# Yuval-H/iclr_17_compression

Hardware: AMD Instinct MI355X
Metric: Mpixels/s encode+decode at 1/2/4/8 GPU; bpp & PSNR parity on Kodak (higher is better)
Workload: dtype h3; 1 GPU; eval encode+decode (round quantiser + rate), 64 x 256x256x3 images per GPU, N=192; N=192, image=256x256x3, batch_per_gpu=64, global_batch=64, quant=round, parallelism=dp1 (images sharded by rank, no data-path collective), launch=eager (kernel by kernel)

## Files before the change

iclr_17_compression_amd/csrc/engine_h3.hip:

```cpp
#include <stdio.h>
#include <stdlib.h>
#include <string.h>

#include <atomic>
#include <type_traits>

#include "common.h"
#include "k5_common.h"

namespace iclr17 {
namespace h3k {
using namespace bfm;

__device__ __attribute__((aligned(16))) unsigned g_zero16h[4] = {0u, 0u, 0u, 0u};
__device__ __forceinline__ const void* zero16(int) { return g_zero16h; }

__device__ __forceinline__ void sink4(void* lds_sink) {
  __builtin_amdgcn_global_load_lds((const __attribute__((address_space(1))) void*)g_zero16h,
                                   (__attribute__((address_space(3))) void*)lds_sink, 4, 0, 0);
}

__device__ __forceinline__ f16v mfma32h(const u4& a, const u4& b, const f16v& c) {
  return __builtin_amdgcn_mfma_f32_32x32x16_f16(__builtin_bit_cast(h8v, a),
                                                __builtin_bit_cast(h8v, b), c, 0, 0, 0);
}

enum HEpi : int { HE_GDN = 0, HE_IGDN = 1, HE_QUANT = 2 };

struct HArgs {
  const u16* in;
  const float* img;
  long in_plane;
  const u16* w;
  long w_plane;
  const float* wscale;
  const float* bias;
  const float* beta;
  const u16* gamma_h3;
  const float* gamma_scale;
  float* out;
  float* pre;
  u16* out_h3;
  long out_h3_plane;
  u16* out_x6;
  long out_x6_plane;
  int out_cm;
  int* range;
  int* wide;
  int qmode;
  const float* noise;
  const float* rate;
  const float* rtab;
  float* yhat;
  double* partial;
  int T;
  int B, Hin, Win, Hout, Wout;
  int gh, gw;
  int tiles_x, tiles_y;
};

constexpr int HM_CONV8 = 2;
constexpr int kConv8Steps = 13;

template <int TH>
struct PatchC8 {
  static constexpr int ROWS = 2 * TH + 3;
  static constexpr int ROWB = 640;
  static constexpr int BYTES = ROWS * ROWB;
  __host__ __device__ static constexpr int off(int pr, int pc) {
    return pr * ROWB + (pc & 1) * 320 + (pc >> 1) * 16;
  }
  __host__ __device__ static constexpr int tap8(int t) {
    return t < 25 ? off(t / 5, t % 5) : 0;
  }
};
constexpr int HM_CONV1 = 3;
constexpr int kConv1Steps = 16;
template <int TH>
struct PatchC1 {
  static constexpr int ROWS = 4 * TH + 5;
  static constexpr int ROWB = 160;
  static constexpr int BYTES = 3 * ROWS * ROWB;
  __host__ __device__ static constexpr int rowoff(int g) { return ((g / 9) * ROWS + g % 9) * ROWB; }
  __host__ __device__ static constexpr int gath(int q) {
    return q < 27 ? ((q / 9) * ROWS + q % 9) * ROWB + 16 : -1;
  }
};

template <int MODE, int TH>
struct HPatch {
  using type = Patch<MODE, TH>;
};
template <int TH>
struct HPatch<HM_CONV8, TH> {
  using type = PatchC8<TH>;
};
template <int TH>
struct HPatch<HM_CONV1, TH> {
  using type = PatchC1<TH>;
};

template <int MODE, int TH, int CO, int CI, bool INT_IN, int NS = 4>
struct HK {
  static constexpr int NW = TH / 2, NTHR = NW * 64;
  static constexpr int NT = CO / 32;
  static constexpr bool C1 = MODE == HM_CONV1;
  static constexpr int CCH = MODE == HM_CONV8 ? 8 : 16;
  static constexpr int NCH = C1 ? 1 : CI / CCH;
  using P = typename HPatch<MODE, TH>::type;
  static constexpr int PL = INT_IN ? 1 : 2;
  static constexpr int PB = PL * P::BYTES;
  static constexpr int NQI = C1 ? 0 : (PB + 1023) / 1024;
  static constexpr int PBUF = (PB + 1023) / 1024 * 1024;
  static constexpr int NPB = C1 ? 1 : 2;
  static constexpr int SB = 2 * 2 * CO * 16;
  static constexpr int NBI = SB / 1024;
  static constexpr int NST = NS;
  static constexpr int MAIN = NPB * PBUF + NST * SB + 1024;
  static constexpr int NTH = NT / 2;
  static constexpr int KB = CO / 16;
  static constexpr int GBL = 2 * NTH * KB;
  static constexpr int LDS0 = MAIN > GBL * 1024 ? MAIN : GBL * 1024;
  static constexpr int BBOFF = (LDS0 + 1023) / 1024 * 1024;
  static constexpr int LDS = BBOFF + 2048 + 256;
  static_assert(SB % 1024 == 0, "weight stage");
  static_assert(C1 || CI % CCH == 0, "tile shape");
  static_assert(LDS <= 160 * 1024, "LDS");
};

__device__ __forceinline__ long h3_out_off(const HArgs& a, int b, int oy, int ox, int CO, int ch) {
  const int cm = a.out_cm;
  if (cm == 0) return (((long)b * a.Hout + oy) * a.Wout + ox) * CO + ch;
  const int sh = __builtin_ctz(cm);
  return ((((long)b * (CO >> sh) + (ch >> sh)) * a.Hout + oy) * a.Wout + ox << sh) + (ch & (cm - 1));
}
__device__ __forceinline__ long h3_out_step32(const HArgs& a) {
  return a.out_cm == 0 ? 32L : 32L * a.Hout * a.Wout;
}

template <int TH, int CO, int COT>
__device__ __forceinline__ void quant_epilogue(const HArgs& a, f16v (&acc)[COT / 32],
                                               unsigned char* lds0, unsigned char* scratch, int b,
                                               int ty, int tx, int cg) {
  constexpr int NT = COT / 32, NW = TH / 2;
  const int etid = fresh_tid(), elane = etid & 63, er32 = elane & 31, eh = elane >> 5;
  const int ewave = __builtin_amdgcn_readfirstlane(etid >> 6);
  const int gy = ty * TH + 2 * ewave + (er32 >> 4), gx = tx * 16 + (er32 & 15);
  const bool inside = gy < a.gh && gx < a.gw;
  const long o = ((long)b * a.Hout + gy) * a.Wout + gx;
  const float dsc = a.wscale[1];
  const bool round = a.qmode == ICLR17_QUANT_ROUND;
  const bool table = a.rtab != nullptr && round;
  float* const lq = (float*)lds0 + etid * 32;
  float bits = 0.f;
  bool ovf = false, wid = false;
  const bool poison = a.range != nullptr && (*(const volatile int*)a.range & 1) != 0;
#pragma unroll
  for (int i = 0; i < NT; ++i) {
    const int c0 = cg * COT + 32 * i;
    float q[16], bv[16];
    bool slow = false;
#pragma unroll
    for (int r = 0; r < 16; ++r) {
      const int c = c0 + 8 * (r >> 2) + 4 * eh + (r & 3);
      const float y = poison ? __builtin_nanf("") : acc[i][r] * dsc;
      acc[i][r] = y;
      const float yh = round ? rintf(y)
                             : y + (inside ? a.noise[(((long)b * CO + c) * a.Hout + gy) * a.Wout + gx] : 0.f);
      q[r] = yh;
      bv[r] = table ? a.rtab[c * 65 + (int)fminf(fmaxf(yh, -32.f), 32.f) + 32] : 0.f;
      slow |= inside && !(table && fabsf(yh) <= 32.f);
    }
    if (slow) {
#pragma unroll
      for (int r = 0; r < 16; ++r) lq[r] = q[r];
#pragma unroll 1
      for (int r = 0; r < 16; ++r) {
        const float v = lq[r];
        if (!(table && fabsf(v) <= 32.f))
          lq[16 + r] = element_bits(v, a.rate, CO, c0 + 8 * (r >> 2) + 4 * eh + (r & 3));
      }
#pragma unroll
      for (int r = 0; r < 16; ++r)
        if (!(table && fabsf(q[r]) <= 32.f)) bv[r] = lq[16 + r];
    }
#pragma unroll
    for (int r = 0; r < 16; ++r) bits += inside ? bv[r] : 0.f;
    f4 yq[4];
#pragma unroll
    for (int m = 0; m < 4; ++m) {
      yq[m] = f4{q[4 * m], q[4 * m + 1], q[4 * m + 2], q[4 * m + 3]};
      if (inside) {
        *(f4*)(a.yhat + o * CO + c0 + 8 * m + 4 * eh) = yq[m];
        if (a.out)
          *(f4*)(a.out + o * CO + c0 + 8 * m + 4 * eh) =
              f4{acc[i][4 * m], acc[i][4 * m + 1], acc[i][4 * m + 2], acc[i][4 * m + 3]};
      }
    }
    if (a.out_h3) {
      uint2 hb[4], lb[4];
      bool ov = false, wd = false;
#pragma unroll
      for (int m = 0; m < 4; ++m) h3_split4(yq[m], hb[m], lb[m], ov, wd);
      ovf |= inside && ov;
      wid |= inside && wd;
      u4 sv[2][2];
#pragma unroll
      for (int pl = 0; pl < 2; ++pl)
#pragma unroll
        for (int k = 0; k < 2; ++k) {
          const uint2 A = pl ? lb[k] : hb[k], Bv = pl ? lb[k + 2] : hb[k + 2];
          const auto sx = __builtin_amdgcn_permlane32_swap(A.x, Bv.x, false, false);
          const auto sy = __builtin_amdgcn_permlane32_swap(A.y, Bv.y, false, false);
          sv[pl][k] = u4{sx[0], sy[0], sx[1], sy[1]};
        }
      if (inside) {
        const long s0 = h3_out_off(a, b, gy, gx, CO, c0 + 16 * eh);
        const long s1 = h3_out_off(a, b, gy, gx, CO, c0 + 16 * eh + 8);
        *(u4*)(a.out_h3 + s0) = sv[0][0];
        *(u4*)(a.out_h3 + s1) = sv[0][1];
        *(u4*)(a.out_h3 + a.out_h3_plane + s0) = sv[1][0];
        *(u4*)(a.out_h3 + a.out_h3_plane + s1) = sv[1][1];
      }
    }
  }
  if (ovf && a.range) atomicOr(a.range, 2);
  if (wid && a.wide) atomicOr(a.wide, 1);
  bits = wave_sum(poison ? __builtin_nanf("") : bits);
  float* sw = (float*)scratch;
  if (elane == 0) sw[ewave] = bits;
  __syncthreads();
  if (etid == 0) {
    double t = 0.0;
#pragma unroll
    for (int w = 0; w < NW; ++w) t += (double)sw[w];
    a.partial[(long)b * a.T + (ty * a.tiles_x + tx) * (CO / COT) + cg] = t;
  }
}

template <int MODE, int TH, int CO, int CI, int EPI, bool INT_IN, int PH, int COT = CO,
          bool SEP = false, int ICM = 0>
__device__ __forceinline__ void h3k_body(const HArgs& a, unsigned char* smem, int b, int ty, int tx,
                                         int cg, bool narrow) {
  static_assert(CO % COT == 0 && (COT == CO || EPI == HE_QUANT), "channel groups: conv3 only");
  constexpr int NSG = EPI == HE_QUANT ? 6 : 4;
  using KK = HK<MODE, TH, COT, CI, INT_IN, NSG>;
  using P = typename KK::P;
  constexpr bool CONV = MODE != BM_DECONV, C8 = MODE == HM_CONV8, C1 = MODE == HM_CONV1;
  using TP = Taps<CONV ? BM_CONV : BM_DECONV, PH>;
  constexpr int NT = KK::NT, NW = KK::NW, NCH = KK::NCH;
  constexpr int S = C1 ? kConv1Steps : C8 ? kConv8Steps : TP::T;
  constexpr int SB = KK::SB, NBI = KK::NBI, NST = KK::NST;
  const int tid = threadIdx.x, lane = tid & 63;
  const int wave = __builtin_amdgcn_readfirstlane(tid >> 6);
  const int r32 = lane & 31, h = lane >> 5;
  constexpr int F = NSG - 2 < S - 1 ? NSG - 2 : (S >= 3 ? 2 : 1), SI = S - F;
  static_assert(SI >= 1 && NST >= F + 2, "DMA schedule");
  constexpr int PS = (KK::NQI + SI - 1) / SI;
  constexpr int K = (NBI + PS + NW - 1) / NW;
  static_assert(F * K < 64, "vmcnt");
  constexpr int GS = NCH * S;
  unsigned char* const sP = smem;
  unsigned char* const sB = smem + KK::NPB * KK::PBUF;
  unsigned char* const sD = sB + NST * SB;
  float* const sbb = (float*)(smem + KK::BBOFF);
  const long img = (long)b * a.Hin * a.Win;
  const int iy0 = CONV ? 2 * ty * TH - 2 : ty * TH - 1;
  const int ix0 = CONV ? 2 * tx * 16 - 2 : tx * 16 - 1;
  static_assert(ICM == 0 || ICM == KK::CCH, "chunk-major input: one chunk per layout chunk");
  const long cstride = ICM ? (long)a.Hin * a.Win * ICM : KK::CCH;
  constexpr int PXS = ICM ? ICM : CI;
  const u16* __restrict__ inb = a.in + img * CI;
  auto piece_src = [&](int piece) -> long {
    const int byte = (piece * 64 + lane) * 16;
    const int pl = byte / P::BYTES, rem = byte - pl * P::BYTES;
    const int pr = rem / P::ROWB, r1 = rem - pr * P::ROWB;
    int pc, hh = 0;
    bool ok;
    if constexpr (C1) {
      pc = 0;
      ok = false;
    } else if constexpr (C8) {
      const int par = r1 / 320, slot = (r1 - par * 320) / 16;
      pc = 2 * slot + par;
      ok = slot < 18 && pc < 35;
    } else if constexpr (MODE == BM_CONV) {
      const int par = r1 / (2 * P::HALF), r2 = r1 - par * 2 * P::HALF;
      hh = r2 / P::HALF;
      pc = 2 * ((r2 - hh * P::HALF) / 16) + par;
      ok = pc < 35;
    } else {
      hh = r1 / P::HALF;
      pc = (r1 - hh * P::HALF) / 16;
      ok = true;
    }
    const int iy = iy0 + pr, ix = ix0 + pc;
    ok = ok && pl < KK::PL && (unsigned)iy < (unsigned)a.Hin && (unsigned)ix < (unsigned)a.Win;
    return ok ? pl * a.in_plane + (long)(iy * a.Win + ix) * PXS + 8 * hh : -1;
  };
  auto issue_piece = [&](int c1, int piece, bool valid) {
    if (!valid) {
      sink4(sD);
      return;
    }
    const long src = piece_src(piece);
    glds16(src >= 0 ? (const void*)(inb + src + c1 * cstride) : zero16(lane),
           sP + (c1 & 1) * KK::PBUF + piece * 1024);
  };
  constexpr long WSTEP = 2L * CO * 8;
  const u16* __restrict__ wph = a.w;
  if (MODE == BM_DECONV) {
    long off = 0;
#pragma unroll
    for (int p = 0; p < PH; ++p) {
      const int ny = (p >> 1) == 0 ? 3 : 2, nx = (p & 1) == 0 ? 3 : 2;
      off += (long)NCH * ny * nx * WSTEP;
    }
    wph += off;
  }
  int wsrc[K];
#pragma unroll
  for (int k = 0; k < K; ++k) {
    const int q = (k * NW + wave) * 64 + lane;
    const int pl = q / (2 * COT), u = q - pl * (2 * COT), hu = u / COT;
    wsrc[k] = (int)(pl * a.w_plane) + (hu * CO + cg * COT + (u - hu * COT)) * 8;
  }
  auto issue_w = [&](int k, int wg) {
    const int slot = k * NW + wave;
    if (wg >= GS) {
      sink4(sD);
      return;
    }
    glds16(wph + (long)wg * WSTEP + wsrc[k], sB + (wg % NST) * SB + slot * 1024);
  };

  const int prow = 2 * wave + (r32 >> 4), pcol = r32 & 15;
  const int tpix = prow * 16 + pcol;
  int pbase;
  if constexpr (C1) pbase = 4 * prow * P::ROWB + 8 * pcol;
  else if constexpr (C8) pbase = P::off(2 * prow, 2 * pcol);
  else pbase = (MODE == BM_CONV ? P::off(2 * prow, 2 * pcol) : P::off(prow, pcol)) + h * P::HALF;
  auto tap_of = [&](int s) -> int {
    if constexpr (C8) return h ? P::tap8(2 * s + 1) : P::tap8(2 * s);
    else if constexpr (C1) return 0;
    else return P::template tap_off<PH>(s);
  };
  const int abase = (h * COT + r32) * 16;
  constexpr int APL = 2 * COT * 16;

  f16v acc[NT], cacc[NT];
#pragma unroll
  for (int i = 0; i < NT; ++i)
#pragma unroll
    for (int j = 0; j < 16; ++j) acc[i][j] = 0.f;

  static_assert(CO <= 256, "bias / β stage");
  if (EPI != HE_QUANT && wave < 2) {
    const float* src = wave == 0 ? a.bias : a.beta;
    glds16(lane * 4 < CO ? (const void*)(src + lane * 4) : zero16(lane), sbb + wave * 256);
  }
  for (int piece = wave; piece < KK::NQI; piece += NW) issue_piece(0, piece, true);
#pragma unroll
  for (int f = 0; f < F; ++f)
#pragma unroll
    for (int k = 0; k < K; ++k)
      if (k * NW + wave < NBI) issue_w(k, f);
#pragma unroll
  for (int k = 0; k < K; ++k) {
    if (k * NW + wave < NBI) issue_w(k, F);
    else sink4(sD);
  }
#pragma unroll
  for (int f = 1; f < F; ++f)
#pragma unroll
    for (int k = 0; k < K; ++k) sink4(sD);
  if constexpr (C1) {
    constexpr int QR = 18, NU = 3 * P::ROWS * QR, IT = (NU + KK::NTHR - 1) / KK::NTHR;
    const int jy0 = 4 * TH * ty - 4, jx0 = 64 * tx - 4;
    const float* __restrict__ xb = a.img + (long)b * 3 * a.Hin * a.Win;
    f4 v[IT];
#pragma unroll
    for (int it = 0; it < IT; ++it) {
      const int u = tid + it * KK::NTHR;
      const int q = u % QR, cr = u / QR, c = cr / P::ROWS, r = cr - c * P::ROWS;
      const int iy = jy0 + r, ix = jx0 + 4 * q;
      const bool ok = u < NU && (unsigned)iy < (unsigned)a.Hin && (unsigned)ix < (unsigned)a.Win;
      v[it] = ok ? *(const f4*)(xb + ((long)c * a.Hin + iy) * a.Win + ix) : f4{0.f, 0.f, 0.f, 0.f};
    }
    bool povf = false;
#pragma unroll
    for (int it = 0; it < IT; ++it) {
      const int u = tid + it * KK::NTHR;
      if (u >= NU) break;
      const int q = u % QR, cr = u / QR;
      uint2 hb, lb;
      h3_split4(v[it], hb, lb, povf);
      *(uint2*)(sP + cr * P::ROWB + 8 * q) = hb;
      *(uint2*)(sP + P::BYTES + cr * P::ROWB + 8 * q) = lb;
    }
    if (povf && a.range) atomicOr(a.range, 1);
    __builtin_amdgcn_s_waitcnt(0xC07F);
  }

  typedef const __attribute__((address_space(3))) u4* lu4p;
  auto dma_k = [&](int k, int c, int s, int g) {
    const int slot = k * NW + wave;
    if ((k + 1) * NW <= NBI || slot < NBI) {
      issue_w(k, g + F + 1);
    } else if (s < SI) {
      const int piece = s * PS + slot - NBI;
      issue_piece(c + 1, piece, c + 1 < NCH && piece < KK::NQI);
    } else {
      sink4(sD);
    }
  };
  struct Frag {
    u4 bh, bl, wh[NT], wl[NT];
  };
  typedef unsigned u2e __attribute__((ext_vector_type(2)));
  typedef const __attribute__((address_space(3))) u2e* lu2p;
  typedef const __attribute__((address_space(3))) unsigned short* lu16p;
  auto conv1_b = [&](const unsigned char* pp, int s) -> u4 {
    u4 v = u4{0u, 0u, 0u, 0u};
    if constexpr (!C1) return v;
    else {
    const int g0 = 2 * s, g1 = 2 * s + 1;
    if (g0 < 27) {
      const int ro = h ? (g1 < 27 ? P::rowoff(g1) : P::rowoff(g0)) : P::rowoff(g0);
      const u2e x0 = *(lu2p)(pp + ro), x1 = *(lu2p)(pp + ro + 8);
      v = u4{x0.x, x0.y, x1.x, x1.y};
    }
    if (g1 >= 27) {
      unsigned e[8];
#pragma unroll
      for (int j = 0; j < 8; ++j) {
        const int oa = g0 >= 27 ? P::gath(8 * (g0 - 27) + j) : -1;
        const int ob = P::gath(8 * (g1 - 27) + j);
        const int o = h ? ob : oa;
        const unsigned x = *(lu16p)(pp + (o >= 0 ? o : 0));
        e[j] = o >= 0 ? x : 0u;
      }
      const u4 w = u4{e[0] | (e[1] << 16), e[2] | (e[3] << 16), e[4] | (e[5] << 16), e[6] | (e[7] << 16)};
      if (g0 >= 27) v = w;
      else if (h) v = w;
    }
    return v;
    }
  };
  auto read_frag = [&](Frag& f, const unsigned char* pb, int to, const unsigned char* wb, int s) {
    if constexpr (C1) {
      f.bh = conv1_b(sP + pbase, s);
      f.bl = conv1_b(sP + P::BYTES + pbase, s);
    } else {
      f.bh = *(lu4p)(pb + to);
      if constexpr (!INT_IN) f.bl = *(lu4p)(pb + P::BYTES + to);
      else f.bl = u4{0u, 0u, 0u, 0u};
    }
#pragma unroll
    for (int i = 0; i < NT; ++i) {
      f.wh[i] = *(lu4p)(wb + i * 512);
      f.wl[i] = *(lu4p)(wb + APL + i * 512);
    }
  };
  auto main_loop = [&](auto narrow_form) {
  constexpr bool NARROW = decltype(narrow_form)::value;
  Frag cur;
  int stage = 1;
  for (int c = 0; c < NCH; ++c) {
    if constexpr (SEP) {
#pragma unroll
      for (int i = 0; i < NT; ++i)
#pragma unroll
        for (int j = 0; j < 16; ++j) cacc[i][j] = 0.f;
    }
#pragma unroll
    for (int s = 0; s < S; ++s) {
      const int g = c * S + s;
      wait_vm_barrier<(F - 1) * K>();
      if (s == 0 && c == 0) read_frag(cur, sP + pbase, tap_of(0), sB + abase, 0);
      Frag nxt;
      read_frag(nxt, sP + ((s + 1 < S ? c : c + 1) & 1) * KK::PBUF + pbase,
                tap_of(s + 1 < S ? s + 1 : 0), sB + stage * SB + abase, s + 1 < S ? s + 1 : 0);
      stage = stage + 1 == NST ? 0 : stage + 1;
      u4 bh11 = cur.bh;
      if constexpr (NARROW) bh11 = h3_x2048(cur.bh);
#pragma unroll
      for (int i = 0; i < NT; ++i) {
        f16v t = SEP ? cacc[i] : acc[i];
        if constexpr (!INT_IN) t = mfma32h(cur.wh[i], cur.bl, t);
        t = mfma32h(cur.wl[i], cur.bh, t);
        if constexpr (NARROW) t = mfma32h(cur.wh[i], bh11, t);
        else t = mfma32h(h3_x2048(cur.wh[i]), cur.bh, t);
        if constexpr (SEP) cacc[i] = t;
        else acc[i] = t;
      }
#pragma unroll
      for (int k = 0; k < K; ++k) dma_k(k, c, s, g);
      cur = nxt;
    }
    if constexpr (SEP) {
#pragma unroll
      for (int i = 0; i < NT; ++i) acc[i] += cacc[i];
    }
  }
  };
  if (!C1 && __builtin_amdgcn_readfirstlane((int)narrow)) main_loop(std::true_type{});
  else main_loop(std::false_type{});
  vm_barrier();
  if constexpr (EPI == HE_QUANT) {
    using KF = HK<MODE, TH, COT, CI, false, NSG>;
    static_assert(TH / 2 * 64 * 128 <= KF::BBOFF, "the epilogue's lane rows fit the stages");
    quant_epilogue<TH, CO, COT>(a, acc, smem, smem + KF::BBOFF, b, ty, tx, cg);
    return;
  } else {

  const int etid = fresh_tid(), elane = etid & 63, er32 = elane & 31, eh = elane >> 5;
  const int ewave = __builtin_amdgcn_readfirstlane(etid >> 6);
  const int etpix = (2 * ewave + (er32 >> 4)) * 16 + (er32 & 15);
  const int gy = ty * TH + (etpix >> 4), gx = tx * 16 + (etpix & 15);
  const bool inside = gy < a.gh && gx < a.gw;
  const int oy = CONV ? gy : 2 * gy + (PH >> 1);
  const int ox = CONV ? gx : 2 * gx + (PH & 1);
  const long o = ((long)b * a.Hout + oy) * a.Wout + ox;
  const float dsc = a.wscale[1];
  const long hb0 = h3_out_off(a, b, oy, ox, CO, 16 * eh), hb1 = h3_out_off(a, b, oy, ox, CO, 16 * eh + 8);
  const long hstep = h3_out_step32(a);
#pragma unroll
  for (int i = 0; i < NT; ++i)
#pragma unroll
    for (int m = 0; m < 4; ++m) {
      const f4 bv = *(const f4*)(sbb + 32 * i + 8 * m + 4 * eh);
#pragma unroll
      for (int j = 0; j < 4; ++j) acc[i][4 * m + j] = acc[i][4 * m + j] * dsc + bv[j];
    }
  constexpr int NTH = KK::NTH, KB = KK::KB;
  static_assert(NT % 2 == 0, "GDN epilogue: pairs of 32-channel tiles");
  bool ovf = false, wid = false;
  float mx = 0.f;
#pragma unroll
  for (int i = 0; i < NT; ++i)
#pragma unroll
    for (int j = 0; j < 16; ++j) mx = fmaxf(mx, fabsf(acc[i][j]));
  mx = fmaxf(mx, __shfl_xor(mx, 32, 64));
  int ep = 0;
  {
    const float m2 = mx * mx;
    if (m2 > 0.f && m2 <= 3.40282347e38f) {
      int e;
      frexpf(m2, &e);
      ep = 14 - e < 100 ? 14 - e : 100;
    }
  }
  const float sp = ldexpf(1.0f, ep);
  const float nsc = ldexpf(a.gamma_scale[1] * kH3Sa, -ep);
  constexpr int KH = KB / 2, HBL = 2 * NTH * KH, GK = (HBL + NW - 1) / NW;
  static_assert(KB % 2 == 0 && 2 * HBL * 1024 <= KK::LDS0, "γ half-stages");
  auto stage_g = [&](int q) {
    const int hf = q >> 1, kh = q & 1;
#pragma unroll
    for (int k = 0; k < GK; ++k) {
      const int blk = k * NW + ewave;
      if (blk >= HBL) {
        sink4((unsigned char*)sbb + 2048);
        continue;
      }
      const int p = blk / (NTH * KH), rem = blk - p * NTH * KH;
      const int il = rem / KH, kb = kh * KH + rem - il * KH;
      glds16(a.gamma_h3 + (long)p * CO * CO + ((2 * kb + eh) * CO + 32 * (hf * NTH + il) + er32) * 8,
             smem + (q & 1) * HBL * 1024 + blk * 1024);
    }
  };
  stage_g(0);
  stage_g(1);
#pragma unroll
  for (int hf = 0; hf < 2; ++hf) {
#pragma unroll
    for (int i = 0; i < NT; ++i)
#pragma unroll
      for (int j = 0; j < 16; ++j) asm volatile("" : "+v"(acc[i][j]));
    f16v n[NTH];
#pragma unroll
    for (int il = 0; il < NTH; ++il)
#pragma unroll
      for (int j = 0; j < 16; ++j) n[il][j] = 0.f;
#pragma unroll
    for (int kh = 0; kh < 2; ++kh) {
      const int q = 2 * hf + kh;
      if (q == 0) {
        wait_vm_barrier<GK>();
      } else {
        vm_barrier();
        if (q + 1 < 4 && q >= 1) stage_g(q + 1);
      }
      const unsigned char* sg = smem + (q & 1) * HBL * 1024 + elane * 16;
#pragma unroll
      for (int kk = 0; kk < KH; ++kk) {
        const int kb = kh * KH + kk;
        const int i = kb >> 1, r0 = 8 * (kb & 1);
        unsigned hv[4], lv[4];
#pragma unroll
        for (int qq = 0; qq < 4; ++qq) {
          typedef float f2 __attribute__((ext_vector_type(2)));
          const f2 v = f2{acc[i][r0 + 2 * qq] * acc[i][r0 + 2 * qq], acc[i][r0 + 2 * qq + 1] * acc[i][r0 + 2 * qq + 1]} * sp;
          const h2v hh = __builtin_convertvector(v, h2v);
          const h2v ll = __builtin_convertvector((v - __builtin_convertvector(hh, f2)) * 2048.0f, h2v);
          hv[qq] = __builtin_bit_cast(unsigned, hh);
          lv[qq] = __builtin_bit_cast(unsigned, ll);
        }
        u4 xp[2];
#pragma unroll
        for (int pl = 0; pl < 2; ++pl) {
          const unsigned* v = pl == 0 ? hv : lv;
          const auto s0 = __builtin_amdgcn_permlane32_swap(v[0], v[2], false, false);
          const auto s1 = __builtin_amdgcn_permlane32_swap(v[1], v[3], false, false);
          xp[pl] = u4{s0[0], s1[0], s0[1], s1[1]};
        }
#pragma unroll
        for (int il = 0; il < NTH; ++il) {
          const u4 gh = *(lu4p)(sg + ((0 * NTH + il) * KH + kk) * 1024);
          const u4 gl = *(lu4p)(sg + ((1 * NTH + il) * KH + kk) * 1024);
          f16v t = mfma32h(gh, xp[1], n[il]);
          t = mfma32h(gl, xp[0], t);
          n[il] = mfma32h(h3_x2048(gh), xp[0], t);
        }
        __builtin_amdgcn_sched_barrier(0);
      }
    }
#pragma unroll
    for (int il = 0; il < NTH; ++il)
#pragma unroll
      for (int j = 0; j < 16; ++j) n[il][j] = n[il][j] * nsc;
#pragma unroll
    for (int il = 0; il < NTH; ++il) {
      const int i = hf * NTH + il;
      f4 y[4], bes[4];
#pragma unroll
      for (int m = 0; m < 4; ++m) bes[m] = *(const f4*)(sbb + 256 + 32 * i + 8 * m + 4 * eh);
#pragma unroll
      for (int m = 0; m < 4; ++m) {
        const int ch = 32 * i + 8 * m + 4 * eh;
        if (inside && a.pre)
          *(f4*)(a.pre + o * CO + ch) = f4{acc[i][4 * m], acc[i][4 * m + 1], acc[i][4 * m + 2], acc[i][4 * m + 3]};
        const f4 be = bes[m];
#pragma unroll
        for (int j = 0; j < 4; ++j) {
          const float nn = n[il][4 * m + j] + be[j];
          const float x = acc[i][4 * m + j];
          y[m][j] = EPI == HE_IGDN ? x * __builtin_amdgcn_sqrtf(nn) : x * __builtin_amdgcn_rsqf(nn);
        }
        if (inside && a.out) *(f4*)(a.out + o * CO + ch) = y[m];
      }
      if (a.out_h3) {
        uint2 hb[4], lb[4];
        bool ov = false, wd = false;
#pragma unroll
        for (int m = 0; m < 4; ++m) h3_split4(y[m], hb[m], lb[m], ov, wd);
        ovf |= inside && ov;
        wid |= inside && wd;
        u4 sv[2][2];
#pragma unroll
        for (int pl = 0; pl < 2; ++pl)
#pragma unroll
          for (int k = 0; k < 2; ++k) {
            const uint2 A = pl ? lb[k] : hb[k], B = pl ? lb[k + 2] : hb[k + 2];
            const auto sx = __builtin_amdgcn_permlane32_swap(A.x, B.x, false, false);
            const auto sy = __builtin_amdgcn_permlane32_swap(A.y, B.y, false, false);
            sv[pl][k] = u4{sx[0], sy[0], sx[1], sy[1]};
          }
        if (inside) {
          const long s0 = hb0 + i * hstep, s1 = hb1 + i * hstep;
          *(u4*)(a.out_h3 + s0) = sv[0][0];
          *(u4*)(a.out_h3 + s1) = sv[0][1];
          *(u4*)(a.out_h3 + a.out_h3_plane + s0) = sv[1][0];
          *(u4*)(a.out_h3 + a.out_h3_plane + s1) = sv[1][1];
        }
      }
      if (a.out_x6) {
        uint2 xp[3][4];
#pragma unroll
        for (int m = 0; m < 4; ++m) {
          unsigned hb[4], mb[4], lb[4];
#pragma unroll
          for (int j = 0; j < 4; ++j) {
            hb[j] = __float_as_uint(y[m][j]) & 0xffff0000u;
            const float r = y[m][j] - __uint_as_float(hb[j]);
            mb[j] = __float_as_uint(r) & 0xffff0000u;
            lb[j] = __float_as_uint(r - __uint_as_float(mb[j]));
          }
          xp[0][m] = uint2{__builtin_amdgcn_perm(hb[1], hb[0], 0x07060302u), __builtin_amdgcn_perm(hb[3], hb[2], 0x07060302u)};
          xp[1][m] = uint2{__builtin_amdgcn_perm(mb[1], mb[0], 0x07060302u), __builtin_amdgcn_perm(mb[3], mb[2], 0x07060302u)};
          xp[2][m] = uint2{__builtin_amdgcn_perm(lb[1], lb[0], 0x07060302u), __builtin_amdgcn_perm(lb[3], lb[2], 0x07060302u)};
        }
        u4 sv6[3][2];
#pragma unroll
        for (int pl = 0; pl < 3; ++pl)
#pragma unroll
          for (int k = 0; k < 2; ++k) {
            const auto sx = __builtin_amdgcn_permlane32_swap(xp[pl][k].x, xp[pl][k + 2].x, false, false);
            const auto sy = __builtin_amdgcn_permlane32_swap(xp[pl][k].y, xp[pl][k + 2].y, false, false);
            sv6[pl][k] = u4{sx[0], sy[0], sx[1], sy[1]};
          }
        if (inside) {
          const long so = o * CO + 32 * i + 16 * eh;
#pragma unroll
          for (int pl = 0; pl < 3; ++pl) {
            *(u4*)(a.out_x6 + pl * a.out_x6_plane + so) = sv6[pl][0];
            *(u4*)(a.out_x6 + pl * a.out_x6_plane + so + 8) = sv6[pl][1];
          }
        }
      }
    }
  }
  if (ovf && a.range) atomicOr(a.range, 1);
  if (wid && a.wide) atomicOr(a.wide, 1);
  }
}

template <int MODE, int TH, int CO, int CI, int EPI, bool INT_OK, int COT = CO, bool SEP = false,
          int ICM = 0>
__global__ void __launch_bounds__(TH / 2 * 64, TH == 8 && MODE != BM_DECONV ? 2 : 1)
h3k_kernel(const HArgs a) {
  constexpr int NSG = EPI == HE_QUANT ? 6 : 4;
  using KK = HK<MODE, TH, COT, CI, false, NSG>;
  static_assert(KK::LDS >= HK<MODE, TH, COT, CI, true, NSG>::LDS, "LDS");
  __shared__ __attribute__((aligned(16))) unsigned char smem[KK::LDS];
  int bid = blockIdx.x;
  const int per_ph = a.tiles_x * a.tiles_y * a.B;
  const int ph = MODE == BM_DECONV ? bid / per_ph : 0;
  bid -= ph * per_ph;
  const int cg = bid % (CO / COT);
  bid /= CO / COT;
  const int tx = bid % a.tiles_x;
  bid /= a.tiles_x;
  const int ty = bid % a.tiles_y;
  const int b = bid / a.tiles_y;
  const bool narrow = a.wide != nullptr && *(const volatile int*)a.wide == 0;
  bool small = false;
  if constexpr (INT_OK) {
    static_assert(MODE == BM_DECONV, "INT_OK: deconv1");
    using P = Patch<MODE, TH>;
    constexpr int COLS = MODE == BM_CONV ? 35 : 18, PER = COLS * CI / 8;
    const int iy0 = MODE == BM_CONV ? 2 * ty * TH - 2 : ty * TH - 1;
    const int ix0 = MODE == BM_CONV ? 2 * tx * 16 - 2 : tx * 16 - 1;
    const u16* inb = a.in + a.in_plane + (long)b * a.Hin * a.Win * CI;
    constexpr int NTHR = TH / 2 * 64, IT = (P::ROWS * PER + NTHR - 1) / NTHR, IB = 8;
    unsigned bad = 0;
#pragma unroll
    for (int i0 = 0; i0 < IT; i0 += IB) {
      u4 v[IB];
#pragma unroll
      for (int k = 0; k < IB; ++k) {
        const int u = threadIdx.x + (i0 + k) * NTHR;
        int r, c;
        long off;
        if constexpr (ICM != 0) {
          constexpr int PR = COLS * ICM / 8;
          const int q = u / (P::ROWS * PR), rem = u - q * (P::ROWS * PR);
          r = rem / PR;
          const int rem2 = rem - r * PR;
          c = rem2 / (ICM / 8);
          off = (((long)q * a.Hin + iy0 + r) * a.Win + ix0 + c) * ICM + 8 * (rem2 - c * (ICM / 8));
        } else {
          r = u / PER;
          const int rem = u - r * PER;
          c = rem / (CI / 8);
          off = ((long)(iy0 + r) * a.Win + ix0 + c) * CI + 8 * (rem - c * (CI / 8));
        }
        const int iy = iy0 + r, ix = ix0 + c;
        const bool ok = i0 + k < IT && u < P::ROWS * PER && (unsigned)iy < (unsigned)a.Hin &&
                        (unsigned)ix < (unsigned)a.Win;
        v[k] = ok ? *(const u4*)(inb + off) : u4{0u, 0u, 0u, 0u};
      }
#pragma unroll
      for (int k = 0; k < IB; ++k)
#pragma unroll
        for (int e = 0; e < 4; ++e) bad |= v[k][e] & 0x7fff7fffu;
    }
    small = __syncthreads_or(bad) == 0;
  }
  auto run = [&](auto int_in) {
    constexpr bool II = decltype(int_in)::value;
    if constexpr (MODE != BM_DECONV) {
      h3k_body<MODE, TH, CO, CI, EPI, II, 0, COT, SEP, ICM>(a, smem, b, ty, tx, cg, narrow);
    } else {
      switch (ph) {
        case 0: h3k_body<MODE, TH, CO, CI, EPI, II, 0, CO, false, ICM>(a, smem, b, ty, tx, 0, narrow); break;
        case 1: h3k_body<MODE, TH, CO, CI, EPI, II, 1, CO, false, ICM>(a, smem, b, ty, tx, 0, narrow); break;
        case 2: h3k_body<MODE, TH, CO, CI, EPI, II, 2, CO, false, ICM>(a, smem, b, ty, tx, 0, narrow); break;
        default: h3k_body<MODE, TH, CO, CI, EPI, II, 3, CO, false, ICM>(a, smem, b, ty, tx, 0, narrow); break;
      }
    }
  };
  if (INT_OK && small) run(std::true_type{});
  else run(std::false_type{});
}

constexpr unsigned kAbsmaxSlots = 256;
__device__ unsigned g_absmax_slot[kAbsmaxSlots][2];

__device__ __forceinline__ void absmax_body(const float* __restrict__ w, long n,
                                            float* __restrict__ trailer, unsigned slot, int bx,
                                            int nbx) {
  __shared__ bool last;
  __shared__ float wmax[4];
  float m = 0.f;
  const long n4 = ((uintptr_t)w & 15) == 0 ? n / 4 : 0;
  for (long i = (long)bx * 256 + threadIdx.x; i < n4; i += (long)nbx * 256) {
    const f4 v = *(const f4*)(w + 4 * i);
    m = fmaxf(m, fmaxf(fmaxf(fabsf(v[0]), fabsf(v[1])), fmaxf(fabsf(v[2]), fabsf(v[3]))));
  }
  for (long i = 4 * n4 + (long)bx * 256 + threadIdx.x; i < n; i += (long)nbx * 256)
    m = fmaxf(m, fabsf(w[i]));
#pragma unroll
  for (int off = 32; off > 0; off >>= 1) m = fmaxf(m, __shfl_xor(m, off, 64));
  if ((threadIdx.x & 63) == 0) wmax[threadIdx.x >> 6] = m;
  __syncthreads();
  unsigned* s = g_absmax_slot[slot];
  if (threadIdx.x == 0) {
    atomicMax(&s[0], __float_as_uint(fmaxf(fmaxf(wmax[0], wmax[1]), fmaxf(wmax[2], wmax[3]))));
    last = __hip_atomic_fetch_add(&s[1], 1u, __ATOMIC_ACQ_REL, __HIP_MEMORY_SCOPE_AGENT) ==
           (unsigned)nbx - 1;
  }
  __syncthreads();
  if (last && threadIdx.x == 0) {
    trailer[0] = __uint_as_float(atomicExch(&s[0], 0u));
    __hip_atomic_store(&s[1], 0u, __ATOMIC_RELAXED, __HIP_MEMORY_SCOPE_AGENT);
  }
}

__global__ void __launch_bounds__(256) absmax_kernel(const float* __restrict__ w, long n,
                                                     float* __restrict__ trailer, unsigned slot) {
  absmax_body(w, n, trailer, slot, blockIdx.x, gridDim.x);
}

static std::atomic<unsigned> g_next_slot{0};
static int absmax_blocks(long n) {
  const long blocks = (n + 16383) / 16384;
  return (int)(blocks < 256 ? (blocks > 0 ? blocks : 1) : 256);
}

static int launch_absmax(const float* w, long n, float* trailer, hipStream_t st) {
  hipLaunchKernelGGL(absmax_kernel, dim3((unsigned)absmax_blocks(n)), dim3(256), 0, st, w, n,
                     trailer, g_next_slot.fetch_add(1) % kAbsmaxSlots);
  return check_launch("absmax");
}

__device__ __forceinline__ int h3_weight_exp(float mx) {
  if (!(mx > 0.f) || !(mx <= 3.40282347e38f)) return 0;
  int e;
  frexpf(mx, &e);
  return 4 - e < 100 ? 4 - e : 100;
}

__device__ __forceinline__ void pack_h3k_body(const float* __restrict__ w, int N, int deconv,
                                              long groups, u16* __restrict__ out,
                                              float* __restrict__ trailer, int bx, int nbx) {
  const int se = h3_weight_exp(trailer[0]);
  const float sw = ldexpf(1.0f, se);
  if (bx == 0 && threadIdx.x == 0) trailer[1] = ldexpf(1.0f, -11 - kH3SaLog2 - se);
  const int nch = N / 16;
  for (long g = (long)bx * 256 + threadIdx.x; g < groups; g += (long)nbx * 256) {
    const int co = (int)(g % N);
    long r = g / N;
    const int h = (int)(r % 2);
    int u = (int)(r / 2);
    int c, ky, kx, ci0;
    bool zero = false;
    if (deconv == 2) {
      c = 0;
      ci0 = 0;
      ky = kx = 0;
      zero = true;
    } else if (!deconv) {
      c = u / kConv8Steps;
      const int t = 2 * (u - c * kConv8Steps) + h;
      zero = t >= 25;
      ky = zero ? 0 : t / 5;
      kx = zero ? 0 : t % 5;
      ci0 = 8 * c;
    } else {
      int p = 0, T = 9;
      while (true) {
        const int ny = (p >> 1) == 0 ? 3 : 2, nx = (p & 1) == 0 ? 3 : 2;
        T = ny * nx;
        if (u < nch * T) break;
        u -= nch * T;
        ++p;
      }
      const int nx = (p & 1) == 0 ? 3 : 2;
      c = u / T;
      const int t = u - c * T;
      ky = (p >> 1) == 0 ? 2 * (t / nx) : 2 * (t / nx) + 1;
      kx = (p & 1) == 0 ? 2 * (t % nx) : 2 * (t % nx) + 1;
      ci0 = 16 * c + 8 * h;
    }
    unsigned short hv[8], lv[8];
#pragma unroll
    for (int j = 0; j < 8; ++j) {
      const int ci = ci0 + j;
      float v;
      if (deconv == 2) {
        const int g = 2 * u + h;
        int cc = -1, yy = 0, xx = 0;
        if (g < 27) {
          cc = g / 9; yy = g % 9; xx = j;
        } else {
          const int q = 8 * (g - 27) + j;
          if (q < 27) { cc = q / 9; yy = q % 9; xx = 8; }
        }
        v = cc < 0 ? 0.f : w[(((long)co * 3 + cc) * 9 + yy) * 9 + xx] * sw;
      } else {
        v = zero ? 0.f
                 : (deconv ? w[(((long)ci * N + co) * 5 + ky) * 5 + kx]
                           : w[(((long)co * N + ci) * 5 + ky) * 5 + kx]) * sw;
      }
      const _Float16 hh = (_Float16)v;
      hv[j] = h16_bits(hh);
      lv[j] = h16_bits((_Float16)((v - (float)hh) * 2048.0f));
    }
    u4 H, L;
#pragma unroll
    for (int i = 0; i < 4; ++i) {
      H[i] = hv[2 * i] | ((unsigned)hv[2 * i + 1] << 16);
      L[i] = lv[2 * i] | ((unsigned)lv[2 * i + 1] << 16);
    }
    *(u4*)(out + g * 8) = H;
    *(u4*)(out + groups * 8 + g * 8) = L;
  }
}

__global__ void __launch_bounds__(256) pack_h3k_kernel(const float* __restrict__ w, int N, int deconv,
                                                       long groups, u16* __restrict__ out,
                                                       float* __restrict__ trailer) {
  pack_h3k_body(w, N, deconv, groups, out, trailer, blockIdx.x, gridDim.x);
}

__device__ __forceinline__ void split_packed_h3_body(const float* __restrict__ w, int K, int N,
                                                     long groups, u16* __restrict__ out,
                                                     float* __restrict__ trailer, int bx, int nbx) {
  const int se = h3_weight_exp(trailer[0]);
  const float sw = ldexpf(1.0f, se);
  if (bx == 0 && threadIdx.x == 0) trailer[1] = ldexpf(1.0f, -11 - kH3SaLog2 - se);
  for (long g = (long)bx * 256 + threadIdx.x; g < groups; g += (long)nbx * 256) {
    const long tk = g / N;
    const int col = (int)(g - tk * N);
    const long tap = tk / (K / 8);
    const int k8 = (int)(tk - tap * (K / 8));
    const float* src = w + ((tap * (K / 4) + 2 * k8) * N + col) * 4;
    const f4 x0 = *(const f4*)src, x1 = *(const f4*)(src + (long)N * 4);
// ... 420 lines not shown
```

Baseline: 3637 Mpix/s.

## Compute GDN norm for all output tiles in one pass, parking accumulators in LDS

Previously the GDN epilogue ran the gamma matmul in two halves, each over all k, which meant forming the squared activations twice. Now a single pass over four k-quarters accumulates the norm for all NT tiles at once. For the TH=16, NT=6 case, two accumulator tiles are parked in LDS and swapped back in when needed, to keep register pressure down. The nsc scale is folded into an FMA with beta. This halves the squaring, splitting and permlane work, at the cost of more live norm accumulators and extra LDS traffic and space.

```diff
diff --git a/iclr_17_compression_amd/csrc/engine_h3.hip b/iclr_17_compression_amd/csrc/engine_h3.hip
--- a/iclr_17_compression_amd/csrc/engine_h3.hip
+++ b/iclr_17_compression_amd/csrc/engine_h3.hip
@@ -117,10 +117,13 @@
   static constexpr int NBI = SB / 1024;
   static constexpr int NST = NS;
   static constexpr int MAIN = NPB * PBUF + NST * SB + 1024;
-  static constexpr int NTH = NT / 2;
   static constexpr int KB = CO / 16;
-  static constexpr int GBL = 2 * NTH * KB;
-  static constexpr int LDS0 = MAIN > GBL * 1024 ? MAIN : GBL * 1024;
+  static constexpr int KQ = KB / 4;
+  static constexpr int GBL = 2 * NT * KQ;
+  static constexpr int NPK = TH == 16 && NT == 6 ? 2 : 0;
+  static constexpr int PKOFF = 2 * GBL * 1024;
+  static constexpr int EPIB = PKOFF + NPK * NW * 4096;
+  static constexpr int LDS0 = MAIN > EPIB ? MAIN : EPIB;
   static constexpr int BBOFF = (LDS0 + 1023) / 1024 * 1024;
   static constexpr int LDS = BBOFF + 2048 + 256;
   static_assert(SB % 1024 == 0, "weight stage");
@@ -525,6 +528,24 @@
   const float dsc = a.wscale[1];
   const long hb0 = h3_out_off(a, b, oy, ox, CO, 16 * eh), hb1 = h3_out_off(a, b, oy, ox, CO, 16 * eh + 8);
   const long hstep = h3_out_step32(a);
+  constexpr int KB = KK::KB, KQ = KK::KQ, QBL = KK::GBL, GK = (QBL + NW - 1) / NW, NPK = KK::NPK;
+  static_assert(KB % 4 == 0 && NT % 2 == 0, "GDN epilogue: k-quarters, pairs of k-blocks per tile");
+  auto stage_g = [&](int q) {
+#pragma unroll
+    for (int k = 0; k < GK; ++k) {
+      const int blk = k * NW + ewave;
+      if (blk >= QBL) {
+        sink4((unsigned char*)sbb + 2048);
+        continue;
+      }
+      const int p = blk / (NT * KQ), rem = blk - p * NT * KQ;
+      const int i = rem / KQ, kb = q * KQ + rem - i * KQ;
+      glds16(a.gamma_h3 + (long)p * CO * CO + ((2 * kb + eh) * CO + 32 * i + er32) * 8,
+             smem + (q & 1) * QBL * 1024 + blk * 1024);
+    }
+  };
+  stage_g(0);
+  stage_g(1);
 #pragma unroll
   for (int i = 0; i < NT; ++i)
 #pragma unroll
@@ -533,8 +554,6 @@
 #pragma unroll
       for (int j = 0; j < 4; ++j) acc[i][4 * m + j] = acc[i][4 * m + j] * dsc + bv[j];
     }
-  constexpr int NTH = KK::NTH, KB = KK::KB;
-  static_assert(NT % 2 == 0, "GDN epilogue: pairs of 32-channel tiles");
   bool ovf = false, wid = false;
   float mx = 0.f;
 #pragma unroll
@@ -553,86 +572,94 @@
   }
   const float sp = ldexpf(1.0f, ep);
   const float nsc = ldexpf(a.gamma_scale[1] * kH3Sa, -ep);
-  constexpr int KH = KB / 2, HBL = 2 * NTH * KH, GK = (HBL + NW - 1) / NW;
-  static_assert(KB % 2 == 0 && 2 * HBL * 1024 <= KK::LDS0, "γ half-stages");
-  auto stage_g = [&](int q) {
-    const int hf = q >> 1, kh = q & 1;
-#pragma unroll
-    for (int k = 0; k < GK; ++k) {
-      const int blk = k * NW + ewave;
-      if (blk >= HBL) {
-        sink4((unsigned char*)sbb + 2048);
-        continue;
-      }
-      const int p = blk / (NTH * KH), rem = blk - p * NTH * KH;
-      const int il = rem / KH, kb = kh * KH + rem - il * KH;
-      glds16(a.gamma_h3 + (long)p * CO * CO + ((2 * kb + eh) * CO + 32 * (hf * NTH + il) + er32) * 8,
-             smem + (q & 1) * HBL * 1024 + blk * 1024);
-    }
-  };
-  stage_g(0);
-  stage_g(1);
-#pragma unroll
-  for (int hf = 0; hf < 2; ++hf) {
-#pragma unroll
-    for (int i = 0; i < NT; ++i)
-#pragma unroll
-      for (int j = 0; j < 16; ++j) asm volatile("" : "+v"(acc[i][j]));
-    f16v n[NTH];
-#pragma unroll
-    for (int il = 0; il < NTH; ++il)
-#pragma unroll
-      for (int j = 0; j < 16; ++j) n[il][j] = 0.f;
-#pragma unroll
-    for (int kh = 0; kh < 2; ++kh) {
-      const int q = 2 * hf + kh;
-      if (q == 0) {
-        wait_vm_barrier<GK>();
-      } else {
-        vm_barrier();
-        if (q + 1 < 4 && q >= 1) stage_g(q + 1);
-      }
-      const unsigned char* sg = smem + (q & 1) * HBL * 1024 + elane * 16;
-#pragma unroll
-      for (int kk = 0; kk < KH; ++kk) {
-        const int kb = kh * KH + kk;
-        const int i = kb >> 1, r0 = 8 * (kb & 1);
-        unsigned hv[4], lv[4];
-#pragma unroll
-        for (int qq = 0; qq < 4; ++qq) {
-          typedef float f2 __attribute__((ext_vector_type(2)));
-          const f2 v = f2{acc[i][r0 + 2 * qq] * acc[i][r0 + 2 * qq], acc[i][r0 + 2 * qq + 1] * acc[i][r0 + 2 * qq + 1]} * sp;
-          const h2v hh = __builtin_convertvector(v, h2v);
-          const h2v ll = __builtin_convertvector((v - __builtin_convertvector(hh, f2)) * 2048.0f, h2v);
-          hv[qq] = __builtin_bit_cast(unsigned, hh);
-          lv[qq] = __builtin_bit_cast(unsigned, ll);
+  typedef __attribute__((address_space(3))) f4* lf4p;
+  unsigned char* const pk = smem + KK::PKOFF + ewave * 4096 + elane * 16;
+  static_assert(NPK <= NT - NPK, "parked tiles change places with the first ones");
+  if constexpr (NPK > 0) {
+    static_assert(KK::EPIB <= KK::BBOFF, "parked tiles below the bias / β stage");
+#pragma unroll
+    for (int s = 0; s < NPK; ++s)
+#pragma unroll
+      for (int m = 0; m < 4; ++m) {
+        const f16v& t = acc[NT - NPK + s];
+        *(lf4p)(pk + (s * NW * 4 + m) * 1024) = f4{t[4 * m], t[4 * m + 1], t[4 * m + 2], t[4 * m + 3]};
+      }
+  }
+  f16v n[NT];
+#pragma unroll
+  for (int i = 0; i < NT; ++i)
+#pragma unroll
+    for (int j = 0; j < 16; ++j) n[i][j] = 0.f;
+#pragma unroll
+  for (int q = 0; q < 4; ++q) {
+    if (q == 0) {
+      wait_vm_barrier<GK>();
+    } else {
+      vm_barrier();
+      if (q + 1 < 4) stage_g(q + 1);
+    }
+    const unsigned char* sg = smem + (q & 1) * QBL * 1024 + elane * 16;
+#pragma unroll
+    for (int kk = 0; kk < KQ; ++kk) {
+      const int kb = q * KQ + kk;
+      const int i = kb >> 1, r0 = 8 * (kb & 1);
+      if constexpr (NPK > 0) {
+        if (r0 == 0 && i >= NT - NPK) {
+          const int s = i - (NT - NPK);
+#pragma unroll
+          for (int m = 0; m < 4; ++m) {
+            const lf4p row = (lf4p)(pk + (s * NW * 4 + m) * 1024);
+            const f4 t = *row;
+            *row = f4{acc[s][4 * m], acc[s][4 * m + 1], acc[s][4 * m + 2], acc[s][4 * m + 3]};
+#pragma unroll
+            for (int j = 0; j < 4; ++j) acc[i][4 * m + j] = t[j];
+          }
         }
-        u4 xp[2];
-#pragma unroll
-        for (int pl = 0; pl < 2; ++pl) {
-          const unsigned* v = pl == 0 ? hv : lv;
-          const auto s0 = __builtin_amdgcn_permlane32_swap(v[0], v[2], false, false);
-          const auto s1 = __builtin_amdgcn_permlane32_swap(v[1], v[3], false, false);
-          xp[pl] = u4{s0[0], s1[0], s0[1], s1[1]};
+      }
+      unsigned hv[4], lv[4];
+#pragma unroll
+      for (int qq = 0; qq < 4; ++qq) {
+        typedef float f2 __attribute__((ext_vector_type(2)));
+        const f2 v = f2{acc[i][r0 + 2 * qq] * acc[i][r0 + 2 * qq], acc[i][r0 + 2 * qq + 1] * acc[i][r0 + 2 * qq + 1]} * sp;
+        const h2v hh = __builtin_convertvector(v, h2v);
+        const h2v ll = __builtin_convertvector((v - __builtin_convertvector(hh, f2)) * 2048.0f, h2v);
+        hv[qq] = __builtin_bit_cast(unsigned, hh);
+        lv[qq] = __builtin_bit_cast(unsigned, ll);
+      }
+      u4 xp[2];
+#pragma unroll
+      for (int pl = 0; pl < 2; ++pl) {
+        const unsigned* v = pl == 0 ? hv : lv;
+        const auto s0 = __builtin_amdgcn_permlane32_swap(v[0], v[2], false, false);
+        const auto s1 = __builtin_amdgcn_permlane32_swap(v[1], v[3], false, false);
+        xp[pl] = u4{s0[0], s1[0], s0[1], s1[1]};
+      }
+#pragma unroll
+      for (int il = 0; il < NT; ++il) {
+        const u4 gh = *(lu4p)(sg + ((0 * NT + il) * KQ + kk) * 1024);
+        const u4 gl = *(lu4p)(sg + ((1 * NT + il) * KQ + kk) * 1024);
+        f16v t = mfma32h(gh, xp[1], n[il]);
+        t = mfma32h(gl, xp[0], t);
+        n[il] = mfma32h(h3_x2048(gh), xp[0], t);
+      }
+      __builtin_amdgcn_sched_barrier(0);
+    }
+  }
+  asm volatile("" ::: "memory");
+  {
+#pragma unroll
+    for (int io = 0; io < NT; ++io) {
+      const int i = io + NPK < NT ? io + NPK : io + NPK - NT, il = i;
+      if constexpr (NPK > 0) {
+        if (i < NPK) {
+#pragma unroll
+          for (int m = 0; m < 4; ++m) {
+            const f4 t = *(lf4p)(pk + (i * NW * 4 + m) * 1024);
+#pragma unroll
+            for (int j = 0; j < 4; ++j) acc[i][4 * m + j] = t[j];
+          }
         }
-#pragma unroll
-        for (int il = 0; il < NTH; ++il) {
-          const u4 gh = *(lu4p)(sg + ((0 * NTH + il) * KH + kk) * 1024);
-          const u4 gl = *(lu4p)(sg + ((1 * NTH + il) * KH + kk) * 1024);
-          f16v t = mfma32h(gh, xp[1], n[il]);
-          t = mfma32h(gl, xp[0], t);
-          n[il] = mfma32h(h3_x2048(gh), xp[0], t);
-        }
-        __builtin_amdgcn_sched_barrier(0);
-      }
-    }
-#pragma unroll
-    for (int il = 0; il < NTH; ++il)
-#pragma unroll
-      for (int j = 0; j < 16; ++j) n[il][j] = n[il][j] * nsc;
-#pragma unroll
-    for (int il = 0; il < NTH; ++il) {
-      const int i = hf * NTH + il;
+      }
       f4 y[4], bes[4];
 #pragma unroll
       for (int m = 0; m < 4; ++m) bes[m] = *(const f4*)(sbb + 256 + 32 * i + 8 * m + 4 * eh);
@@ -644,7 +671,7 @@
         const f4 be = bes[m];
 #pragma unroll
         for (int j = 0; j < 4; ++j) {
-          const float nn = n[il][4 * m + j] + be[j];
+          const float nn = __builtin_fmaf(n[il][4 * m + j], nsc, be[j]);
           const float x = acc[i][4 * m + j];
           y[m][j] = EPI == HE_IGDN ? x * __builtin_amdgcn_sqrtf(nn) : x * __builtin_amdgcn_rsqf(nn);
         }
```

After: 3683 Mpix/s (median of 6 runs). 1.3% higher.
